# BarclayII/audiogan

Hardware: AMD Instinct MI355X
Metric: audio-samples/sec per G+D train step (8 kHz, 8192-sample clips) (higher is better)
Workload: dtype f32; 1 GPU; C2: full audiogan.py Conv1d/LSTM G + D, batch 64 per GPU, 8192-sample white-noise clips, frame_size 256 (T=32), canonical G+D step, adam, per-parameter clip d=1 g=0.1; global_batch=64, clip_len=8192, parallelism=dp1, launch=hipGraph replay (1 graph per step)

## Files before the change

### audiogan_amd/_lib.py

```python
import ctypes as C
import os

_HERE = os.path.dirname(os.path.abspath(__file__))
LIB_PATH = os.path.join(_HERE, 'libaudiogan_hip.so')

AG_OK, AG_ERR_ARG, AG_ERR_LAUNCH, AG_ERR_UNSUPPORTED = 0, -1, -2, -3
ACT_NONE, ACT_LEAKY, ACT_TANH, ACT_LEAKY_GATE = 0, 1, 2, 3
OPT_RMSPROP, OPT_ADAM = 0, 1
FLAG_NAN, FLAG_BIG = 1, 2

vp, i32, i64, f32 = C.c_void_p, C.c_int32, C.c_int64, C.c_float


class WnDesc(C.Structure):
    _fields_ = [('v', vp), ('g', vp), ('w', vp), ('wpa', vp), ('wpb', vp), ('inv_norm', vp),
                ('rows', i32), ('cols', i32), ('d1', i32), ('K', i32), ('stride', i32), ('pad_', i32)]


class WnBwdDesc(C.Structure):
    _fields_ = [('v', vp), ('g', vp), ('dw', vp), ('dv', vp), ('dg', vp), ('rows', i32), ('cols', i32),
                ('accumulate', i32), ('pad_', i32)]


class ConvArgs(C.Structure):
    _fields_ = [('x', vp), ('wp', vp), ('bias', vp), ('res', vp), ('y', vp), ('lens_i64', vp),
                ('x_bs', i64), ('x_cs', i64), ('y_bs', i64), ('y_cs', i64), ('res_bs', i64),
                ('res_cs', i64), ('B', i32), ('C', i32), ('Lin', i32), ('O', i32), ('Lout', i32),
                ('K', i32), ('stride', i32), ('pad', i32), ('mode', i32), ('act', i32),
                ('slope', f32), ('accumulate', i32), ('wp_pad', i32)]


class FrontFwdArgs(C.Structure):
    _fields_ = [('struct_bytes', i64), ('cell', i32), ('gen', i32)] + [(n, vp) for n in (
        'gates', 'gh', 'w_x', 'w_hh', 'b_hn', 'w_p', 'b_p', 'hs', 'cs', 'x', 'xt', 'w_s', 'b_s', 'u', 's', 'first', 't_run',
        'ws')] + [(n, i64) for n in ('ldx', 'lds', 'ws_bytes')] + [(n, i32) for n in ('ldwx', 'T', 'B', 'S', 'fs', 'n_cu')]


class FrontBwdArgs(C.Structure):
    _fields_ = [('struct_bytes', i64), ('cell', i32), ('pad_', i32)] + [(n, vp) for n in (
        'ga', 'state', 'gh', 'x', 'dh_ext', 'dx_ext', 'w_hh', 'w_x', 'w_p', 'dgs', 'dgh', 'dxt', 'ws')] + [
        (n, i64) for n in ('ldx', 'lddx', 'ws_bytes')] + [(n, i32) for n in ('ldwx', 'T', 'B', 'S', 'fs', 'n_cu')]


class OptDesc(C.Structure):
# ... 12 lines not shown
    'ag_abi_version': (C.c_int, []),
    'ag_bce_logits_fwd_strided': (C.c_int, [vp, i64, i64, C.c_float, vp, vp, vp, vp, C.c_float, C.c_int, C.c_int, vp]),
    'ag_bce_logits_bwd_strided': (C.c_int, [vp, i64, i64, C.c_float, vp, vp, vp, C.c_float, vp, i64, i64, C.c_int, C.c_int, vp]),
    'ag_transpose_batched': (C.c_int, [vp, C.c_int, i64, i64, vp, C.c_int, i64, i64, C.c_int, C.c_int, C.c_int, vp]),
    'ag_defer_reduces': (C.c_int, [C.c_int]),
    'ag_flush_reduces': (C.c_int, [vp]),
    'ag_arch': (C.c_char_p, []),
    'ag_last_error': (C.c_char_p, []),
    'ag_last_kernel': (C.c_char_p, []),
    'ag_weight_norm_fwd': (C.c_int, [vp, C.c_int, C.c_int, vp]),
    'ag_weight_norm_bwd': (C.c_int, [vp, C.c_int, C.c_int, vp]),
    'ag_conv1d_engine': (C.c_int, [C.POINTER(ConvArgs), vp]),
    'ag_prep_conv_weight': (C.c_int, [vp, vp, vp, C.c_int, C.c_int, C.c_int, C.c_int, C.c_int, vp]),
    'ag_wpa_numel': (i64, [C.c_int, C.c_int, C.c_int]),
    'ag_wpb_numel': (i64, [C.c_int, C.c_int, C.c_int, C.c_int]),
    'ag_conv1d_wgrad': (C.c_int, [vp, i64, i64, vp, i64, i64, vp] + [C.c_int] * 8 + [vp]),
    'ag_conv1d_o1_fwd': (C.c_int, [vp, i64, i64, vp, vp, vp, i64, C.c_int, C.c_int, C.c_int, C.c_int, C.c_int,
                                   C.c_int, f32, vp]),
    'ag_conv1d_o1_bwd_data': (C.c_int, [vp, i64, vp, vp, i64, i64, C.c_int, C.c_int, C.c_int, C.c_int, C.c_int,
                                        C.c_int, vp]),
    'ag_conv1d_o1_wgrad': (C.c_int, [vp, i64, vp, i64, i64, vp, C.c_int, C.c_int, C.c_int, C.c_int, C.c_int, vp]),
    'ag_channel_sum': (C.c_int, [vp, i64, i64, vp, C.c_int, C.c_int, C.c_int, C.c_int, vp]),
    'ag_lstm_front_bwd_step': (C.c_int, [vp, C.c_int, vp, C.c_int, vp, C.c_int, C.c_int, vp, vp, C.c_int, vp, vp, vp,
                                         vp, vp, vp, C.c_int, C.c_int, vp]),
    'ag_leaky_bwd': (C.c_int, [vp, i64, i64, vp, i64, i64, vp, i64, i64, vp, i64, i64, vp, vp, C.c_int,
                               C.c_int, C.c_int, f32, vp]),
    'ag_gemm': (C.c_int, [vp, C.c_int, C.c_int, vp, C.c_int, C.c_int, vp, C.c_int, C.c_int,
                          C.c_int, C.c_int, f32, f32, vp, vp, C.c_int, C.c_int, f32, vp]),
    'ag_col_sum': (C.c_int, [vp, C.c_int, C.c_int, vp, C.c_int, C.c_int, C.c_int, vp]),
    'ag_lstm_cell_fwd': (C.c_int, [vp, C.c_int, vp, C.c_int, vp, C.c_int, vp, C.c_int, vp, C.c_int,
# ... 100 lines not shown
```

### audiogan_amd/common.py

```python
import torch

from . import kernels as K

PARAM_EPOCH = [0]


CAPTURE_EPOCH = [0]


def new_capture():
    CAPTURE_EPOCH[0] += 1
    return CAPTURE_EPOCH[0]


def capture_tag(dev):
    if torch.device(dev).type == 'cuda' and torch.cuda.is_current_stream_capturing():
        return CAPTURE_EPOCH[0]
    return None


def param_epoch(p):
    return getattr(p, '_ag_epoch', 0)


# ... 87 lines not shown


class Prepared(object):
    __slots__ = ('w', 'wpa', 'wpb', 'pad')

    def __init__(self, w=None, wpa=None, wpb=None, pad=0):
        self.w, self.wpa, self.wpb, self.pad = w, wpa, wpb, pad


class WNGroup(object):

    def __init__(self):
        self.items = []
        self._bufs = None
        self._key = None

    def add(self, v, g, stride=1, engine=False, pad=0):
        self.items.append(dict(v=v, g=g, stride=stride, engine=engine, pad=pad))
        return len(self.items) - 1

    def params(self):
        out = []
        for it in self.items:
            out += [it['v'], it['g']]
        return out

    def _alloc(self, dev):
        bufs = []
        for it in self.items:
            v = it['v']
# ... 15 lines not shown

    def _entries(self):
        return [dict(v=it['v'].data, g=it['g'].data.view(-1), w=p.w, wpa=p.wpa, wpb=p.wpb, stride=it['stride'],
                     pad=it.get('pad', 0)) for it, p in zip(self.items, self._bufs)]

    def prepare(self):
        key = self._current_key()
        if key != self._key:
            K.weight_norm_fwd(self._entries())
            self._mark_fresh(key)
        return self._bufs

    def _mark_fresh(self, key):
        self._key = key
        self._w16 = {}

    def w16(self, i):
        d = getattr(self, '_w16', None)
        if d is None:
            d = self._w16 = {}
        img = d.get(i)
        if img is None:
            keep = getattr(self, '_w16_buf', None)
            if keep is None:
                keep = self._w16_buf = {}
            img = d[i] = K.to_bf16(self._bufs[i].w, out=keep.get(i))
            keep[i] = img
        return img

    def zero_dws(self):
# ... 79 lines not shown
```

### audiogan_amd/csrc/conv_engine.hip

```cpp
#include "conv_engine_impl.h"

int ag_conv_cfg_1214(ConvP& p, hipStream_t st);
int ag_conv_cfg_2114(ConvP& p, hipStream_t st);
int ag_conv_cfg_1122(ConvP& p, hipStream_t st);
int ag_conv_cfg_2122(ConvP& p, hipStream_t st);
int ag_conv_cfg_2222(ConvP& p, hipStream_t st);
int ag_conv_cfg_1141(ConvP& p, hipStream_t st);

extern "C" int64_t ag_wpa_numel(int d0, int d1, int K) {
  const int cp2 = ag_roundup(d1, 2), mp = ag_roundup(d0, 32);
  return ag_wq_offset(cp2, K, mp) + ag_wq_floats(cp2, K, mp);
}
extern "C" int64_t ag_wpb_numel(int d0, int d1, int K, int stride) {
  const int cp2 = ag_roundup(d0, 2), mt = ag_cdiv(K, stride), mp = ag_roundup(d1 * stride, 32);
  return ag_wq_offset(cp2, mt, mp) + ag_wq_floats(cp2, mt, mp);
}

template <typename MainFn, typename TailFn>
static int main_and_tail(hipStream_t st, MainFn mainf, TailFn tailf) {
  const int rc = mainf(st);
  if (rc != AG_OK) return rc;
  const char* main_name = ag_last_kernel();
  const int rt = tailf(st);
  ag_note_kernel(main_name);
  return rt;
}

extern "C" int ag_conv1d_engine(const ag_conv_args* args, void* stream) {
  AG_REQUIRE(args != nullptr, "ag_conv1d_engine: null args");
  ConvP p;
  p.a = *args;
  const ag_conv_args& a = p.a;
  p.aligned = 0;
  p.rb = ag_precision() == AG_PREC_BF16;
  AG_REQUIRE(a.x && a.wp && a.y, "ag_conv1d_engine: null tensor");
  AG_REQUIRE(a.B > 0 && a.C > 0 && a.O > 0 && a.Lin > 0 && a.Lout > 0, "ag_conv1d_engine: bad shape");
  AG_REQUIRE(a.K > 0 && a.stride > 0 && a.pad >= 0, "ag_conv1d_engine: bad conv params");
  AG_REQUIRE(a.B <= 65535, "ag_conv1d_engine: batch > 65535");
  AG_REQUIRE(a.mode == 0 || a.mode == 1, "ag_conv1d_engine: bad mode");
  if (a.mode == 0) {
    p.taps = a.K;
    p.sp = a.stride;
    p.Mrows = a.O;
    p.n_lo = 0;
    p.n_cnt = a.Lout;
    AG_REQUIRE((int64_t)(a.Lout - 1) * a.stride - a.pad < a.Lin, "ag_conv1d_engine: Lout too large");
  } else {
    p.taps = ag_cdiv(a.K, a.stride);
    p.sp = 1;
    p.Mrows = a.O * a.stride;
    if (a.wp_pad == a.pad && ag_scatter_aligned(a.K, a.stride, a.pad)) {
      p.aligned = 1;
      p.n_lo = ag_cdiv(a.pad, a.stride);
      p.n_cnt = ag_cdiv(a.Lout, a.stride);
    } else {
      p.n_lo = a.pad / a.stride;
      const int n_hi = (a.Lout - 1 + a.pad) / a.stride;
      p.n_cnt = n_hi - p.n_lo + 1;
    }
  }
  if (ag_conv_c1_enabled()) {
    int rc = AG_OK;
    if (ag_conv_c1_try_fwd(a, p.rb, (hipStream_t)stream, &rc)) return rc;
    if (ag_conv_c1_try_bwdx(a, p.rb, (hipStream_t)stream, &rc)) return rc;
  }
  AG_REQUIRE(p.taps <= MAX_TAPS, "ag_conv1d_engine: more than %d taps", MAX_TAPS);
  p.sp_shift = ilog2_exact(p.sp);
  p.s_shift = ilog2_exact(a.stride);
  p.efast = (int64_t)a.O * a.y_cs * 4 < ((int64_t)1 << 31) && (!a.res || (int64_t)a.O * a.res_cs * 4 < ((int64_t)1 << 31));
  p.xvec = (((uintptr_t)a.x & 15) == 0) && (a.x_bs % 4 == 0) && (a.x_cs % 4 == 0);
  p.Cpad = ag_roundup(a.C, 2);
  p.Mpad = ag_roundup(p.Mrows, 32);
  hipStream_t st = (hipStream_t)stream;
  if (p.Mrows <= 32) return ag_conv_cfg_1214(p, st);
  const int tail0 = p.n_cnt % 128;
  const int tail = (p.n_cnt - tail0) / 128 < 8 ? tail0 : 0, main_cols = p.n_cnt - tail;
  if (p.Mrows <= 64) {
    if (tail > 0 && tail <= 32 && main_cols > 0) {
      ConvP qm = p, qt = p;
      qm.n_cnt = main_cols;
      qt.n_lo += main_cols;
      qt.n_cnt = tail;
      return main_and_tail(st, [&](hipStream_t s_) { return ag_conv_cfg_2114(qm, s_); },
                           [&](hipStream_t s_) { return ag_conv_cfg_1122(qt, s_); });
// ... 51 lines not shown
}

extern "C" int ag_prep_conv_weight(const float* w, float* wpa, float* wpb, int d0, int d1, int K,
                                   int stride, int pad, void* stream) {
  AG_REQUIRE(w && (wpa || wpb), "ag_prep_conv_weight: null tensor");
  AG_REQUIRE(d0 > 0 && d1 > 0 && K > 0 && stride > 0, "ag_prep_conv_weight: bad shape");
  int64_t n = 0;
  if (wpa) n = ag_wq_offset(ag_roundup(d1, 2), K, ag_roundup(d0, 32));
  const int64_t nbw = ag_wq_offset(ag_roundup(d0, 2), ag_cdiv(K, stride), ag_roundup(d1 * stride, 32));
  if (wpb && nbw > n) n = nbw;
  hipLaunchKernelGGL(prep_conv_weight_kernel, dim3((unsigned)ag_cdiv64(n, 256)), dim3(256), 0,
                     (hipStream_t)stream, w, wpa, wpb, d0, d1, K, stride, pad);
  AG_CHECK_LAUNCH("ag_prep_conv_weight");
  return AG_OK;
}
```

### audiogan_amd/csrc/conv_engine_impl.h

```cpp
#pragma once
#include "common.h"
#include <type_traits>

#define MAX_TAPS 32

struct ConvP {
  ag_conv_args a;
  int taps;
  int sp;
  int sp_shift;
  int ncols;
  int rowlen;
  int chs;
  int CC;
  int Cpad;
  int Mrows;
  int Mpad;
  int n_lo;
  int n_cnt;
  int xvec;
  int aligned;
  int efast;
  int s_shift;
  int ncols_tile;
// ... 14 lines not shown
                                                   int b, int row0, int n0, int wrow0, int wcol0, int l31, int h) {
  const ag_conv_args& a = p.a;
  if (!p.efast) return false;
  const unsigned OOB = 0x80000000u;
  const int ycs = (int)a.y_cs, rcs = (int)a.res_cs;
  int lenb = 0x7fffffff;
  if (a.lens_i64) {
    const int64_t l = a.lens_i64[b];
    lenb = l > 0x7fffffff ? 0x7fffffff : (int)l;
  }
  __amdgpu_buffer_rsrc_t yr = __builtin_amdgcn_make_buffer_rsrc(a.y + (int64_t)b * a.y_bs, 0, (int)((int64_t)a.O * a.y_cs * 4), 0x00020000);
  __amdgpu_buffer_rsrc_t rr = __builtin_amdgcn_make_buffer_rsrc(
      const_cast<float*>(a.res ? a.res + (int64_t)b * a.res_bs : a.y), 0, a.res ? (int)((int64_t)a.O * a.res_cs * 4) : 0, 0x00020000);
  const bool has_res = a.res != nullptr;
  const bool gate = a.act == AG_ACT_LEAKY_GATE;
  if (a.mode == 0) {
#pragma unroll
    for (int i = 0; i < TILES_O; ++i) {
#pragma unroll
      for (int e = 0; e < 16; ++e) {
        const int ro = wrow0 + 32 * i + (e & 3) + 8 * (e >> 2) + 4 * h;
        const int o = row0 + ro;
        const bool valid = o < p.Mrows;
        const float bo = bias_s[ro];
        const int rowy = o * ycs, rowr = o * rcs;
#pragma unroll
        for (int j = 0; j < TILES_T; ++j) {
          const int t = n0 + wcol0 + 32 * j + l31;
          const bool ok = valid && t < a.Lout;
          const unsigned yo = ok ? (unsigned)((rowy + t) * 4) : OOB;
          float v = acc[i][j][e] + bo;
// ... 4 lines not shown
          v = ag_apply_act(v, a.act, a.slope);
          if (t >= lenb) v = 0.f;
          if (a.accumulate) v += __uint_as_float(__builtin_amdgcn_raw_buffer_load_b32(yr, yo, 0, 0));
          __builtin_amdgcn_raw_buffer_store_b32(__float_as_uint(v), yr, yo, 0, 0);
        }
      }
    }
    return true;
  }
  const int s = a.stride;
  const int rho = a.pad % s;
  const bool rot4 = p.aligned && s == 4;
  const bool al4 = p.aligned && s % 4 == 0 && rho % 4 == 0;
  const bool sw2 = p.aligned && s == 2;
  if (!sw2 && (s % 4 != 0 || (p.aligned && !rot4 && !al4))) return false;
  {
    const int nlo = n0, nhi = n0 + p.ncols_tile - 1;
    int lo, hi;
    if (sw2) { lo = 2 * nlo - a.pad - 1; hi = 2 * nhi - a.pad + 1; }
    else if (rot4) { lo = 4 * (nlo - 1) - (a.pad - rho); hi = 4 * nhi - (a.pad - rho); }
    else if (p.aligned) { lo = s * (nlo - 1) + rho - a.pad; hi = s * nhi + rho - a.pad; }
    else { lo = s * nlo - a.pad; hi = s * (nhi + 1) - a.pad; }
    if (lo < 0 || hi > a.Lout) return false;
  }
  const bool need_pre = has_res || a.accumulate;
  if (sw2) {
#pragma unroll
    for (int i = 0; i < TILES_O; ++i) {
#pragma unroll
      for (int g = 0; g < 4; ++g) {
// ... 21 lines not shown
            if (u0 >= lenb) v0 = 0.f;
            if (u0 + 1 >= lenb) v1 = 0.f;
            if (a.accumulate) {
              v0 += __uint_as_float(__builtin_amdgcn_raw_buffer_load_b32(yr, yo, 0, 0));
              v1 += __uint_as_float(__builtin_amdgcn_raw_buffer_load_b32(yr, yo + 4u, 0, 0));
            }
            __builtin_amdgcn_raw_buffer_store_b32(__float_as_uint(v0), yr, yo, 0, 0);
            __builtin_amdgcn_raw_buffer_store_b32(__float_as_uint(v1), yr, yo + 4u, 0, 0);
          }
        }
      }
    }
    return true;
  }
  const int rot = rot4 ? rho : 0;
#pragma unroll
  for (int i = 0; i < TILES_O; ++i) {
    unsigned yo[4][TILES_T];
    cu32x4 pre[4][TILES_T];
#pragma unroll
    for (int g = 0; g < 4; ++g) {
      const int rowb = row0 + wrow0 + 32 * i + 8 * g + 4 * h;
      const bool valid = rowb < p.Mrows;
      const int o = p.s_shift >= 0 ? (rowb >> p.s_shift) : rowb / s;
      const int r = rowb - o * s;
      const int rowy = o * ycs, rowr = o * rcs;
#pragma unroll
      for (int j = 0; j < TILES_T; ++j) {
        const int n = n0 + wcol0 + 32 * j + l31;
        const int u0 = rot4 ? 4 * (n - 1) - (a.pad - rho) : s * (n - ((p.aligned && r >= rho) ? 1 : 0)) + r - a.pad;
// ... 39 lines not shown
        }
        __builtin_amdgcn_raw_buffer_store_b128(out, yr, yo[g][j], 0, 0);
      }
    }
  }
  return true;
}

template <int TILES_O, int TILES_T>
__device__ __forceinline__ void conv_epilogue_any(const ConvP& p, f32x16 (&acc)[TILES_O][TILES_T], const float* bias_s,
                                                  int b, int row0, int n0, int wrow0, int wcol0, int l31, int h) {
  const ag_conv_args& a = p.a;
  const int64_t lenb = a.lens_i64 ? a.lens_i64[b] : (int64_t)1 << 60;
  float* yb = a.y + (int64_t)b * a.y_bs;
  const float* rb = a.res ? a.res + (int64_t)b * a.res_bs : nullptr;
  const int s = a.stride;
  const int rho = a.pad % s;
#pragma unroll
  for (int i = 0; i < TILES_O; ++i) {
#pragma unroll
    for (int e = 0; e < 16; ++e) {
      const int ro = wrow0 + 32 * i + (e & 3) + 8 * (e >> 2) + 4 * h;
      const int row = row0 + ro;
      if (row >= p.Mrows) continue;
      const float bo = bias_s[ro];
      const int o = a.mode == 0 ? row : row / s;
      const int r = row - o * s;
#pragma unroll
      for (int j = 0; j < TILES_T; ++j) {
        const int n = n0 + wcol0 + 32 * j + l31;
        const int u = a.mode == 0 ? n : s * (n - ((p.aligned && r >= rho) ? 1 : 0)) + r - a.pad;
        if (u < 0 || u >= a.Lout) continue;
        float v = acc[i][j][e] + bo;
        if (rb) {
          const float rv = rb[(int64_t)o * a.res_cs + u];
          v = a.act == AG_ACT_LEAKY_GATE ? (rv > 0.f ? v : v * a.slope) : v + rv;
        }
        v = ag_apply_act(v, a.act, a.slope);
        if (u >= lenb) v = 0.f;
        float* dst = yb + (int64_t)o * a.y_cs + u;
        if (a.accumulate) v += *dst;
        *dst = v;
      }
    }
  }
}

template <int TILES_O, int TILES_T>
__device__ __forceinline__ void conv_epilogue(const ConvP& p, f32x16 (&acc)[TILES_O][TILES_T], const float* bias_s,
                                              int b, int row0, int n0, int wrow0, int wcol0, int l31, int h) {
  if (!conv_epilogue_fast<TILES_O, TILES_T>(p, acc, bias_s, b, row0, n0, wrow0, wcol0, l31, h))
    conv_epilogue_any<TILES_O, TILES_T>(p, acc, bias_s, b, row0, n0, wrow0, wcol0, l31, h);
}

template <int TILES_O, int TILES_T, int WAVES_O, int WAVES_T, int TAPS, int S0>
__global__ __launch_bounds__(512) __attribute__((amdgpu_waves_per_eu(4, 4))) void conv_engine_kernel(const ConvP p) {
// ... 628 lines not shown
```

### audiogan_amd/kernels.py

```python
import ctypes as C

import torch

from . import _lib
from ._lib import lib, check, ACT_NONE, ACT_LEAKY, ACT_TANH, ACT_LEAKY_GATE, OPT_RMSPROP, OPT_ADAM

LEAKY_SLOPE = 0.01


def _stream():
    return C.c_void_p(torch.cuda.current_stream().cuda_stream)


def _p(t):
    return C.c_void_p(t.data_ptr()) if t is not None else C.c_void_p(0)


def _chk(t, name, dtype=torch.float32):
    if t is None:
        return
    if not t.is_cuda:
        raise RuntimeError('audiogan_amd: %s must be a CUDA (HIP) tensor; there is no CPU path' % name)
    if t.dtype != dtype:
        raise TypeError('audiogan_amd: %s must be %s, got %s' % (name, dtype, t.dtype))
# ... 278 lines not shown


def prep_conv_weight(w, wpa, wpb, stride, pad=0):
    _chk(w, 'w'); _chk(wpa, 'wpa'); _chk(wpb, 'wpb')
    assert w.dim() == 3 and w.is_contiguous()
    d0, d1, K = w.shape
    if wpa is not None:
        assert wpa.numel() == wpa_numel(d0, d1, K)
    if wpb is not None:
        assert wpb.numel() == wpb_numel(d0, d1, K, stride)
    check(lib.ag_prep_conv_weight(_p(w), _p(wpa), _p(wpb), d0, d1, K, stride, int(pad), _stream()),
          'ag_prep_conv_weight')


def conv_engine(x, wp, y, K, stride, pad, mode, bias=None, res=None, lens=None, act=ACT_NONE,
                slope=LEAKY_SLOPE, accumulate=False, wp_pad=0):
    assert act != ACT_LEAKY_GATE or res is not None, 'ACT_LEAKY_GATE needs the saved activation in `res`'
    x_bs, x_cs = _bcl(x, 'x')
    y_bs, y_cs = _bcl(y, 'y')
    _chk(wp, 'wp'); _chk(bias, 'bias'); _chk(lens, 'lens', torch.int64)
    B, Cc, Lin = x.shape
    B2, O, Lout = y.shape
    assert B == B2
    if mode == 0:
        assert wp.numel() == wpa_numel(O, Cc, K), 'gather weight layout does not match shapes'
    else:
        assert wp.numel() == wpb_numel(Cc, O, K, stride), 'scatter weight layout does not match'
    r_bs = r_cs = 0
    if res is not None:
        r_bs, r_cs = _bcl(res, 'res')
        assert tuple(res.shape) == tuple(y.shape)
    if bias is not None:
        assert bias.numel() == O and bias.is_contiguous()
    if lens is not None:
        assert lens.numel() == B and lens.is_contiguous()
    a = _lib.ConvArgs(x.data_ptr(), wp.data_ptr(), _p(bias).value or 0, _p(res).value or 0,
                      y.data_ptr(), _p(lens).value or 0, x_bs, x_cs, y_bs, y_cs, r_bs, r_cs,
                      B, Cc, Lin, O, Lout, K, stride, pad, mode, act, slope, 1 if accumulate else 0, int(wp_pad))
    check(lib.ag_conv1d_engine(C.byref(a), _stream()), 'ag_conv1d_engine')


def conv_wgrad(sh, lg, dw, K, stride, pad):
    sh_bs, sh_cs = _bcl(sh, 'sh')
    lg_bs, lg_cs = _bcl(lg, 'lg')
    _chk(dw, 'dw')
    B, A, Lsh = sh.shape
    B2, Cc, Llg = lg.shape
    assert B == B2 and dw.is_contiguous() and dw.numel() == A * Cc * K
    _ws = _bind_ws(lib.ag_conv1d_wgrad_ws_numel(B, A, Lsh, Cc, K), dw.device)
    check(lib.ag_conv1d_wgrad(_p(sh), sh_bs, sh_cs, _p(lg), lg_bs, lg_cs, _p(dw), B, A, Lsh, Cc, Llg,
                              K, stride, pad, _stream()), 'ag_conv1d_wgrad')


def channel_sum(dy, db, accumulate=True):
# ... 372 lines not shown
            r['bytes'] += by
        cls.records = []
        return out


def _bf16_tag():
    return '<bf16>' if lib.ag_get_precision() == 1 else ''


def _work_gemm(A, B, Cm, ta=False, tb=False, *a_, **kw):
    M, N = Cm.shape
    Kd = A.size(0) if ta else A.size(1)
    return None, 2.0 * M * N * Kd, 4.0 * (M * Kd + N * Kd + M * N)


def _work_conv(x, wp, y, K_, stride, pad, mode, *a_, **kw):
    B, Cc, Lin = x.shape
    _, O, Lout = y.shape
    macs = B * O * Lout * Cc * K_ if mode == 0 else B * Cc * Lin * O * K_
    return None, 2.0 * macs, 4.0 * (x.numel() + y.numel() + O * Cc * K_)


def _work_wgrad(sh, lg, dw, K_, stride, pad):
    B, A, Lsh = sh.shape
    Cc = lg.size(1)
    return None, 2.0 * B * A * Lsh * Cc * K_, 4.0 * (sh.numel() + lg.numel() + dw.numel())


def _call_sig(a, k):
    def one(v):
        if isinstance(v, torch.Tensor):
            return tuple(v.shape), v.stride(), v.dtype, v.data_ptr() % 16
        if isinstance(v, (list, tuple)):
            return tuple(one(e) for e in v)
        return v
# ... 20 lines not shown
        e0, e1 = torch.cuda.Event(enable_timing=True), torch.cuda.Event(enable_timing=True)
        e0.record()
        r = fn(*a, **k)
        e1.record()
        if key is None:
            key = seen[sig] = lib.ag_last_kernel().decode()
        Profiler.records.append((key, fl, by, e0, e1, nl))
        return r
    wrapped.__name__ = name
    wrapped.__doc__ = fn.__doc__
    wrapped.__module__ = __name__
    globals()[name] = wrapped


for _n, _w in (('gemm', _work_gemm), ('conv_engine', _work_conv), ('conv_wgrad', _work_wgrad),
               ('channel_sum', None), ('leaky_bwd', None), ('col_sum', None), ('lstm_cell_fwd', None),
               ('lstm_cell_bwd', None), ('weight_norm_fwd', None), ('weight_norm_bwd', None),
               ('bce_logits_fwd', None), ('bce_logits_bwd', None), ('act_fwd', None), ('act_bwd', None),
               ('axpby', None), ('grad_norms', None), ('opt_step', None)):
    _instrument(_n, _w)


def _al16(t):
    return t.data_ptr() % 16 == 0


def skinny_ok(A, B, tb):
    M, Kd = A.shape
    ok = M <= 256 and Kd % 8 == 0 and A.stride(1) == 1 and A.stride(0) % 4 == 0 and _al16(A)
    if tb:
        ok = ok and B.stride(1) == 1 and B.stride(0) % 4 == 0 and _al16(B)
# ... 753 lines not shown
```

### audiogan_amd/ops.py

```python
import torch

from . import kernels as K
from .kernels import ACT_NONE, ACT_LEAKY, ACT_TANH, ACT_LEAKY_GATE

from .common import PARAM_EPOCH, Prepared, WNGroup, _zeros_like_list


class ConvSpec(object):
    __slots__ = ('kind', 'cin', 'cout', 'K', 'stride', 'pad', 'out_pad')

    def __init__(self, kind, cin, cout, K_, stride, pad, out_pad=0):
        self.kind, self.cin, self.cout, self.K, self.stride, self.pad = kind, cin, cout, K_, stride, pad
        self.out_pad = out_pad

    def out_len(self, lin):
        if self.kind == 'conv':
            return (lin + 2 * self.pad - self.K) // self.stride + 1
        return (lin - 1) * self.stride - 2 * self.pad + self.K + self.out_pad


def _o1(spec):
    return K.conv_o1_ok(spec.kind, spec.cout, spec.K, spec.stride, spec.pad)


# ... 17 lines not shown
    else:
        K.conv_engine(dy, prep.wpa, dx, spec.K, spec.stride, spec.pad, 0, res=gate, lens=lens, act=act, accumulate=accumulate)


def conv_wgrad(spec, x, dy, dw, db):
    if _o1(spec):
        K.conv_o1_wgrad(dy, x, dw, spec.K, spec.pad)
    elif spec.kind == 'conv':
        K.conv_wgrad(dy, x, dw, spec.K, spec.stride, spec.pad)
    else:
        K.conv_wgrad(x, dy, dw, spec.K, spec.stride, spec.pad)
    if db is not None:
        K.channel_sum(dy, db)


class GTrunk(object):

    def __init__(self, bottlenecks, final):
        self.bottlenecks = bottlenecks
        self.final = final
        self.group = WNGroup()
        self.ctot = 1 + sum(d.cout for _, d in bottlenecks)


class GTrunkFn(torch.autograd.Function):
    @staticmethod
    def forward(ctx, x0, trunk, *params):
        B, L = x0.shape
        prep = trunk.group.prepare()
        ctot = trunk.ctot
        if (x0.stride() == (ctot * L, 1) and x0.storage_offset() == 0 and x0.dtype == torch.float32
                and x0.untyped_storage().nbytes() == 4 * B * ctot * L):
            slab = x0.as_strided((B, ctot, L), (ctot * L, L, 1), 0)
        else:
            slab = torch.empty(B, ctot, L, device=x0.device)
            slab[:, 0, :].copy_(x0)
        hids = []
# ... 26 lines not shown
        dy = dy.contiguous().view(B, 1, L)
        wg = any(ctx.needs_input_grad[2:])
        dws = trunk.group.zero_dws() if wg else None
        dslab = torch.empty_like(slab)
        with K.deferred_reduces():
            GTrunkFn._backward_layers(trunk, prep, slab, hids, dy, dslab, dws, wg, ctot)
        grads = trunk.group.backward(dws) if wg else [None] * (2 * len(trunk.group.items))
        dx0 = dslab[:, 0, :] if ctx.needs_input_grad[0] else None
        return (dx0, None) + tuple(grads)

    @staticmethod
    def _backward_layers(trunk, prep, slab, hids, dy, dslab, dws, wg, ctot):
        if wg:
            conv_wgrad(trunk.final, slab, dy, dws[-2], dws[-1])
        conv_bwd_data(trunk.final, prep[-2], dy, dslab, accumulate=False)
        cin = ctot
        for i in reversed(range(len(trunk.bottlenecks))):
            cs, ds = trunk.bottlenecks[i]
            pw, qw = prep[4 * i], prep[4 * i + 2]
            cin -= ds.cout
            out_v = slab[:, cin:cin + ds.cout]
            dout = dslab[:, cin:cin + ds.cout]
            add = dslab[:, cin - ds.cout:cin] if cin >= ds.cout else None
            K.leaky_bwd(dout, out_v, dout, add_into=add, bias_grad=dws[4 * i + 3] if wg else None)
            hid = hids[i]
            if wg:
                conv_wgrad(ds, hid, dout, dws[4 * i + 2], None)
            dhid = torch.empty_like(hid)
            conv_bwd_data(ds, qw, dout, dhid, gate=hid)
            if wg:
                K.channel_sum(dhid, dws[4 * i + 1])
            if wg:
                conv_wgrad(cs, slab[:, :cin], dhid, dws[4 * i], None)
            conv_bwd_data(cs, pw, dhid, dslab[:, :cin], accumulate=True)


class DConvStack(object):
    def __init__(self, specs):
        self.specs = specs
        self.group = WNGroup()


class DConvStackFn(torch.autograd.Function):

    @staticmethod
    def forward(ctx, x, stack, lens_list, *params):
        B, L = x.shape
        ctx.set_materialize_grads(False)
        prep = stack.group.prepare()
# ... 307 lines not shown
```

### include/audiogan_hip.h

```cpp
#ifndef AUDIOGAN_HIP_H
#define AUDIOGAN_HIP_H

#include <stdint.h>

#ifdef __cplusplus
extern "C" {
#endif

#define AG_OK 0
#define AG_ERR_ARG (-1)
#define AG_ERR_LAUNCH (-2)
#define AG_ERR_UNSUPPORTED (-3)

#define AG_ACT_NONE 0
#define AG_ACT_LEAKY 1
#define AG_ACT_TANH 2
#define AG_ACT_LEAKY_GATE 3

int ag_abi_version(void);
const char* ag_arch(void);
const char* ag_last_error(void);
const char* ag_last_kernel(void);

typedef struct ag_wn_desc {
// ... 15 lines not shown

typedef struct ag_wn_bwd_desc {
  const float* v;
  const float* g;
  const float* dw;
  float* dv;
  float* dg;
  int32_t rows;
  int32_t cols;
  int32_t accumulate;
  int32_t pad_;
} ag_wn_bwd_desc;

int ag_weight_norm_bwd(const ag_wn_bwd_desc* descs_dev, int n, int max_rows, void* stream);

typedef struct ag_conv_args {
  const float* x;
  const float* wp;
  const float* bias;
  const float* res;
  float* y;
  const int64_t* lens_i64;
  int64_t x_bs, x_cs;
  int64_t y_bs, y_cs;
  int64_t res_bs, res_cs;
  int32_t B, C, Lin, O, Lout;
  int32_t K, stride, pad;
  int32_t mode;
  int32_t act;
  float slope;
  int32_t accumulate;
  int32_t wp_pad;
} ag_conv_args;

int ag_conv1d_engine(const ag_conv_args* args, void* stream);

int ag_prep_conv_weight(const float* w, float* wpa, float* wpb, int d0, int d1, int K, int stride, int pad,
                        void* stream);
int64_t ag_wpa_numel(int d0, int d1, int K);
int64_t ag_wpb_numel(int d0, int d1, int K, int stride);

int ag_conv1d_wgrad(const float* sh, int64_t sh_bs, int64_t sh_cs, const float* lg, int64_t lg_bs,
                    int64_t lg_cs, float* dw, int B, int A, int Lsh, int C, int Llg, int K,
                    int stride, int pad, void* stream);

int ag_conv1d_o1_fwd(const float* x, int64_t x_bs, int64_t x_cs, const float* w, const float* bias, float* y,
                     int64_t y_bs, int B, int C, int L, int K, int pad, int act, float slope, void* stream);
int ag_conv1d_o1_bwd_data(const float* dy, int64_t dy_bs, const float* w, float* dx, int64_t dx_bs,
                          int64_t dx_cs, int B, int C, int L, int K, int pad, int accumulate, void* stream);
int ag_conv1d_o1_wgrad(const float* dy, int64_t dy_bs, const float* x, int64_t x_bs, int64_t x_cs, float* dw,
                       int B, int C, int L, int K, int pad, void* stream);

int ag_channel_sum(const float* dy, int64_t bs, int64_t cs, float* db, int B, int C, int L, int accumulate,
                   void* stream);

// ... 237 lines not shown
```

Measured before the change: 31.03 million audio-samples/sec.

## Pull dense-trunk input gradients via concatenated weight panels in generator backward

Restructures the generator dense-trunk backward. Each bottleneck used to scatter its input-gradient conv into the growing slab, followed by a separate leaky backward. Now per-slice weight panels are built from all later bottlenecks (rebuilt when weights change), and one conv per output slice pulls the hidden gradients of every later layer. The leaky gate, residual add and pre-accumulate are fused into that conv's epilogue. This cuts repeated read-modify-write passes over the gradient slab and launches, at the cost of extra panel memory, a pull kernel per weight refresh and a new epilogue path that bypasses the c1 fast path.

```diff
diff --git a/audiogan_amd/_lib.py b/audiogan_amd/_lib.py
--- a/audiogan_amd/_lib.py
+++ b/audiogan_amd/_lib.py
@@ -6,6 +6,7 @@
 
 AG_OK, AG_ERR_ARG, AG_ERR_LAUNCH, AG_ERR_UNSUPPORTED = 0, -1, -2, -3
 ACT_NONE, ACT_LEAKY, ACT_TANH, ACT_LEAKY_GATE = 0, 1, 2, 3
+CONV_ACC_POST, CONV_ACC_PRE = 1, 2
 OPT_RMSPROP, OPT_ADAM = 0, 1
 FLAG_NAN, FLAG_BIG = 1, 2
 
@@ -27,7 +28,13 @@
                 ('x_bs', i64), ('x_cs', i64), ('y_bs', i64), ('y_cs', i64), ('res_bs', i64),
                 ('res_cs', i64), ('B', i32), ('C', i32), ('Lin', i32), ('O', i32), ('Lout', i32),
                 ('K', i32), ('stride', i32), ('pad', i32), ('mode', i32), ('act', i32),
-                ('slope', f32), ('accumulate', i32), ('wp_pad', i32)]
+                ('slope', f32), ('accumulate', i32), ('wp_pad', i32), ('gate_from', i32), ('add', vp),
+                ('add_bs', i64), ('add_cs', i64)]
+
+
+class PullDesc(C.Structure):
+    _fields_ = [('src', vp), ('dst', vp), ('C', i32), ('taps', i32), ('src_mp', i32), ('row0', i32), ('rows', i32),
+                ('dst_mp', i32), ('c0', i32), ('ctot', i32)]
 
 
 class FrontFwdArgs(C.Structure):
@@ -70,6 +77,7 @@
     'ag_prep_conv_weight': (C.c_int, [vp, vp, vp, C.c_int, C.c_int, C.c_int, C.c_int, C.c_int, vp]),
     'ag_wpa_numel': (i64, [C.c_int, C.c_int, C.c_int]),
     'ag_wpb_numel': (i64, [C.c_int, C.c_int, C.c_int, C.c_int]),
+    'ag_pull_panels': (C.c_int, [vp, C.c_int, i64, vp]),
     'ag_conv1d_wgrad': (C.c_int, [vp, i64, i64, vp, i64, i64, vp] + [C.c_int] * 8 + [vp]),
     'ag_conv1d_o1_fwd': (C.c_int, [vp, i64, i64, vp, vp, vp, i64, C.c_int, C.c_int, C.c_int, C.c_int, C.c_int,
                                    C.c_int, f32, vp]),
diff --git a/audiogan_amd/common.py b/audiogan_amd/common.py
--- a/audiogan_amd/common.py
+++ b/audiogan_amd/common.py
@@ -125,6 +125,7 @@
         self.items = []
         self._bufs = None
         self._key = None
+        self.derived = None
 
     def add(self, v, g, stride=1, engine=False, pad=0):
         self.items.append(dict(v=v, g=g, stride=stride, engine=engine, pad=pad))
@@ -170,6 +171,9 @@
     def _mark_fresh(self, key):
         self._key = key
         self._w16 = {}
+        derived = getattr(self, 'derived', None)
+        if derived is not None:
+            derived(self._bufs)
 
     def w16(self, i):
         d = getattr(self, '_w16', None)
diff --git a/audiogan_amd/csrc/conv_engine.hip b/audiogan_amd/csrc/conv_engine.hip
--- a/audiogan_amd/csrc/conv_engine.hip
+++ b/audiogan_amd/csrc/conv_engine.hip
@@ -38,6 +38,10 @@
   AG_REQUIRE(a.K > 0 && a.stride > 0 && a.pad >= 0, "ag_conv1d_engine: bad conv params");
   AG_REQUIRE(a.B <= 65535, "ag_conv1d_engine: batch > 65535");
   AG_REQUIRE(a.mode == 0 || a.mode == 1, "ag_conv1d_engine: bad mode");
+  AG_REQUIRE(a.accumulate >= 0 && a.accumulate <= AG_CONV_ACC_PRE, "ag_conv1d_engine: bad accumulate");
+  AG_REQUIRE(a.gate_from >= 0 && a.gate_from <= a.O, "ag_conv1d_engine: gate_from outside the output channels");
+  AG_REQUIRE(a.gate_from == 0 || a.act == AG_ACT_NONE || a.act == AG_ACT_LEAKY_GATE,
+             "ag_conv1d_engine: gate_from needs AG_ACT_LEAKY_GATE or AG_ACT_NONE");
   if (a.mode == 0) {
     p.taps = a.K;
     p.sp = a.stride;
@@ -59,7 +63,7 @@
       p.n_cnt = n_hi - p.n_lo + 1;
     }
   }
-  if (ag_conv_c1_enabled()) {
+  if (ag_conv_c1_enabled() && !a.add) {
     int rc = AG_OK;
     if (ag_conv_c1_try_fwd(a, p.rb, (hipStream_t)stream, &rc)) return rc;
     if (ag_conv_c1_try_bwdx(a, p.rb, (hipStream_t)stream, &rc)) return rc;
@@ -67,7 +71,8 @@
   AG_REQUIRE(p.taps <= MAX_TAPS, "ag_conv1d_engine: more than %d taps", MAX_TAPS);
   p.sp_shift = ilog2_exact(p.sp);
   p.s_shift = ilog2_exact(a.stride);
-  p.efast = (int64_t)a.O * a.y_cs * 4 < ((int64_t)1 << 31) && (!a.res || (int64_t)a.O * a.res_cs * 4 < ((int64_t)1 << 31));
+  p.efast = (int64_t)a.O * a.y_cs * 4 < ((int64_t)1 << 31) && (!a.res || (int64_t)a.O * a.res_cs * 4 < ((int64_t)1 << 31)) &&
+            (!a.add || (int64_t)a.O * a.add_cs * 4 < ((int64_t)1 << 31));
   p.xvec = (((uintptr_t)a.x & 15) == 0) && (a.x_bs % 4 == 0) && (a.x_cs % 4 == 0);
   p.Cpad = ag_roundup(a.C, 2);
   p.Mpad = ag_roundup(p.Mrows, 32);
@@ -149,3 +154,25 @@
   AG_CHECK_LAUNCH("ag_prep_conv_weight");
   return AG_OK;
 }
+
+__global__ __launch_bounds__(256) void pull_panels_kernel(const ag_pull_desc* __restrict__ descs) {
+  const ag_pull_desc d = descs[blockIdx.y];
+  const int64_t i = (int64_t)blockIdx.x * 256 + threadIdx.x;
+  if (i >= (int64_t)d.C * d.taps * d.dst_mp) return;
+  const int row = (int)(i % d.dst_mp);
+  const int cm = (int)(i / d.dst_mp);
+  const int m = cm % d.taps, c = cm / d.taps;
+  const float val = row < d.rows ? d.src[(int64_t)cm * d.src_mp + d.row0 + row] : 0.f;
+  d.dst[((int64_t)(d.c0 + c) * d.taps + m) * d.dst_mp + row] = val;
+  unsigned short* q = reinterpret_cast<unsigned short*>(d.dst + ag_wq_offset((d.ctot + 1) & ~1, d.taps, d.dst_mp));
+  q[ag_wq_index(d.c0 + c, m, row, d.taps, d.dst_mp)] = (unsigned short)ag_pack_bf16(val, val);
+}
+
+extern "C" int ag_pull_panels(const ag_pull_desc* descs_dev, int n, int64_t max_elems, void* stream) {
+  AG_REQUIRE(descs_dev && n > 0 && max_elems > 0, "ag_pull_panels: bad args");
+  AG_REQUIRE(n <= 65535, "ag_pull_panels: too many descriptors");
+  hipLaunchKernelGGL(pull_panels_kernel, dim3((unsigned)ag_cdiv64(max_elems, 256), n), dim3(256), 0,
+                     (hipStream_t)stream, descs_dev);
+  AG_CHECK_LAUNCH("ag_pull_panels");
+  return AG_OK;
+}
diff --git a/audiogan_amd/csrc/conv_engine_impl.h b/audiogan_amd/csrc/conv_engine_impl.h
--- a/audiogan_amd/csrc/conv_engine_impl.h
+++ b/audiogan_amd/csrc/conv_engine_impl.h
@@ -52,7 +52,9 @@
       const_cast<float*>(a.res ? a.res + (int64_t)b * a.res_bs : a.y), 0, a.res ? (int)((int64_t)a.O * a.res_cs * 4) : 0, 0x00020000);
   const bool has_res = a.res != nullptr;
   const bool gate = a.act == AG_ACT_LEAKY_GATE;
+  const bool pull = a.accumulate == AG_CONV_ACC_PRE || a.add != nullptr || a.gate_from > 0;
   if (a.mode == 0) {
+    if (pull) return false;
 #pragma unroll
     for (int i = 0; i < TILES_O; ++i) {
 #pragma unroll
@@ -87,6 +89,7 @@
   const bool al4 = p.aligned && s % 4 == 0 && rho % 4 == 0;
   const bool sw2 = p.aligned && s == 2;
   if (!sw2 && (s % 4 != 0 || (p.aligned && !rot4 && !al4))) return false;
+  if (sw2 && pull) return false;
   {
     const int nlo = n0, nhi = n0 + p.ncols_tile - 1;
     int lo, hi;
@@ -138,6 +141,76 @@
     return true;
   }
   const int rot = rot4 ? rho : 0;
+  if (pull) {
+    __amdgpu_buffer_rsrc_t ar = __builtin_amdgcn_make_buffer_rsrc(
+        const_cast<float*>(a.add ? a.add + (int64_t)b * a.add_bs : a.y), 0, a.add ? (int)((int64_t)a.O * a.add_cs * 4) : 0, 0x00020000);
+    const int acs = (int)a.add_cs;
+    const bool has_add = a.add != nullptr;
+    const bool acc_pre = a.accumulate == AG_CONV_ACC_PRE, acc_post = a.accumulate == AG_CONV_ACC_POST;
+    const cu32x4 zero4 = {0u, 0u, 0u, 0u};
+#pragma unroll
+    for (int i = 0; i < TILES_O; ++i) {
+#pragma unroll
+      for (int gh = 0; gh < 2; ++gh) {
+        unsigned yo[2][TILES_T];
+        cu32x4 pr[2][TILES_T], py[2][TILES_T], pa[2][TILES_T];
+#pragma unroll
+        for (int g2 = 0; g2 < 2; ++g2) {
+          const int rowb = row0 + wrow0 + 32 * i + 8 * (2 * gh + g2) + 4 * h;
+          const bool valid = rowb < p.Mrows;
+          const int o = p.s_shift >= 0 ? (rowb >> p.s_shift) : rowb / s;
+          const int r = rowb - o * s;
+#pragma unroll
+          for (int j = 0; j < TILES_T; ++j) {
+            const int n = n0 + wcol0 + 32 * j + l31;
+            const int u0 = rot4 ? 4 * (n - 1) - (a.pad - rho) : s * (n - ((p.aligned && r >= rho) ? 1 : 0)) + r - a.pad;
+            yo[g2][j] = valid ? (unsigned)((o * ycs + u0) * 4) : OOB;
+            pr[g2][j] = has_res ? __builtin_amdgcn_raw_buffer_load_b128(rr, valid ? (unsigned)((o * rcs + u0) * 4) : OOB, 0, 0) : zero4;
+            py[g2][j] = a.accumulate ? __builtin_amdgcn_raw_buffer_load_b128(yr, yo[g2][j], 0, 0) : zero4;
+            pa[g2][j] = has_add ? __builtin_amdgcn_raw_buffer_load_b128(ar, valid ? (unsigned)((o * acs + u0) * 4) : OOB, 0, 0) : zero4;
+          }
+        }
+#pragma unroll
+        for (int g2 = 0; g2 < 2; ++g2) {
+          const int g = 2 * gh + g2;
+          const int ro = wrow0 + 32 * i + 8 * g + 4 * h;
+          const int rowb = row0 + ro;
+          const int o = p.s_shift >= 0 ? (rowb >> p.s_shift) : rowb / s;
+          const int r = rowb - o * s;
+          const float bo = bias_s[ro];
+          const bool gated = o >= a.gate_from;
+#pragma unroll
+          for (int j = 0; j < TILES_T; ++j) {
+            const int n = n0 + wcol0 + 32 * j + l31;
+            const int u0 = rot4 ? 4 * (n - 1) - (a.pad - rho) : s * (n - ((p.aligned && r >= rho) ? 1 : 0)) + r - a.pad;
+            const float v4[4] = {acc[i][j][4 * g], acc[i][j][4 * g + 1], acc[i][j][4 * g + 2], acc[i][j][4 * g + 3]};
+            float v[4];
+            if (rot == 0) { v[0] = v4[0]; v[1] = v4[1]; v[2] = v4[2]; v[3] = v4[3]; }
+            else if (rot == 1) { v[0] = v4[1]; v[1] = v4[2]; v[2] = v4[3]; v[3] = v4[0]; }
+            else if (rot == 2) { v[0] = v4[2]; v[1] = v4[3]; v[2] = v4[0]; v[3] = v4[1]; }
+            else { v[0] = v4[3]; v[1] = v4[0]; v[2] = v4[1]; v[3] = v4[2]; }
+            cu32x4 out;
+#pragma unroll
+            for (int q = 0; q < 4; ++q) {
+              const float rv = __uint_as_float(pr[g2][j][q]), ov = __uint_as_float(py[g2][j][q]);
+              float w = v[q] + bo;
+              if (has_res && !gate) w += rv;
+              if (acc_pre) w += ov;
+              if (has_add) w += __uint_as_float(pa[g2][j][q]);
+              if (gated) {
+                w = gate ? (rv > 0.f ? w : w * a.slope) : ag_apply_act(w, a.act, a.slope);
+                if (u0 + q >= lenb) w = 0.f;
+              }
+              if (acc_post) w += ov;
+              out[q] = __float_as_uint(w);
+            }
+            __builtin_amdgcn_raw_buffer_store_b128(out, yr, yo[g2][j], 0, 0);
+          }
+        }
+      }
+    }
+    return true;
+  }
 #pragma unroll
   for (int i = 0; i < TILES_O; ++i) {
     unsigned yo[4][TILES_T];
@@ -207,6 +280,8 @@
   const int64_t lenb = a.lens_i64 ? a.lens_i64[b] : (int64_t)1 << 60;
   float* yb = a.y + (int64_t)b * a.y_bs;
   const float* rb = a.res ? a.res + (int64_t)b * a.res_bs : nullptr;
+  const float* ab = a.add ? a.add + (int64_t)b * a.add_bs : nullptr;
+  const bool gate = a.act == AG_ACT_LEAKY_GATE;
   const int s = a.stride;
   const int rho = a.pad % s;
 #pragma unroll
@@ -225,14 +300,16 @@
         const int u = a.mode == 0 ? n : s * (n - ((p.aligned && r >= rho) ? 1 : 0)) + r - a.pad;
         if (u < 0 || u >= a.Lout) continue;
         float v = acc[i][j][e] + bo;
-        if (rb) {
-          const float rv = rb[(int64_t)o * a.res_cs + u];
-          v = a.act == AG_ACT_LEAKY_GATE ? (rv > 0.f ? v : v * a.slope) : v + rv;
-        }
-        v = ag_apply_act(v, a.act, a.slope);
-        if (u >= lenb) v = 0.f;
         float* dst = yb + (int64_t)o * a.y_cs + u;
-        if (a.accumulate) v += *dst;
+        const float rv = rb ? rb[(int64_t)o * a.res_cs + u] : 0.f;
+        if (rb && !gate) v += rv;
+        if (a.accumulate == AG_CONV_ACC_PRE) v += *dst;
+        if (ab) v += ab[(int64_t)o * a.add_cs + u];
+        if (o >= a.gate_from) {
+          v = gate ? (rv > 0.f ? v : v * a.slope) : ag_apply_act(v, a.act, a.slope);
+          if (u >= lenb) v = 0.f;
+        }
+        if (a.accumulate == AG_CONV_ACC_POST) v += *dst;
         *dst = v;
       }
     }
diff --git a/audiogan_amd/kernels.py b/audiogan_amd/kernels.py
--- a/audiogan_amd/kernels.py
+++ b/audiogan_amd/kernels.py
@@ -4,6 +4,7 @@
 
 from . import _lib
 from ._lib import lib, check, ACT_NONE, ACT_LEAKY, ACT_TANH, ACT_LEAKY_GATE, OPT_RMSPROP, OPT_ADAM
+from ._lib import CONV_ACC_POST, CONV_ACC_PRE
 
 LEAKY_SLOPE = 0.01
 
@@ -316,7 +317,7 @@
 
 
 def conv_engine(x, wp, y, K, stride, pad, mode, bias=None, res=None, lens=None, act=ACT_NONE,
-                slope=LEAKY_SLOPE, accumulate=False, wp_pad=0):
+                slope=LEAKY_SLOPE, accumulate=False, wp_pad=0, add=None, gate_from=0):
     assert act != ACT_LEAKY_GATE or res is not None, 'ACT_LEAKY_GATE needs the saved activation in `res`'
     x_bs, x_cs = _bcl(x, 'x')
     y_bs, y_cs = _bcl(y, 'y')
@@ -336,10 +337,32 @@
         assert bias.numel() == O and bias.is_contiguous()
     if lens is not None:
         assert lens.numel() == B and lens.is_contiguous()
+    a_bs = a_cs = 0
+    if add is not None:
+        a_bs, a_cs = _bcl(add, 'add')
+        assert tuple(add.shape) == tuple(y.shape)
+    assert 0 <= gate_from <= O and (gate_from == 0 or act in (ACT_NONE, ACT_LEAKY_GATE))
     a = _lib.ConvArgs(x.data_ptr(), wp.data_ptr(), _p(bias).value or 0, _p(res).value or 0,
                       y.data_ptr(), _p(lens).value or 0, x_bs, x_cs, y_bs, y_cs, r_bs, r_cs,
-                      B, Cc, Lin, O, Lout, K, stride, pad, mode, act, slope, 1 if accumulate else 0, int(wp_pad))
+                      B, Cc, Lin, O, Lout, K, stride, pad, mode, act, slope, int(accumulate), int(wp_pad),
+                      int(gate_from), _p(add).value or 0, a_bs, a_cs)
     check(lib.ag_conv1d_engine(C.byref(a), _stream()), 'ag_conv1d_engine')
+
+
+def pull_panels(entries):
+    descs, nmax = [], 1
+    for e in entries:
+        _chk(e['src'], 'src'); _chk(e['dst'], 'dst')
+        Cc, taps, smp, dmp, ctot = e['C'], e['taps'], e['src_mp'], e['dst_mp'], e['ctot']
+        cp2 = (ctot + 1) // 2 * 2
+        assert 0 <= e['row0'] and e['row0'] + e['rows'] <= smp and e['rows'] <= dmp and e['c0'] + Cc <= ctot
+        assert e['src'].numel() >= Cc * taps * smp, 'source layout smaller than its descriptor'
+        assert e['dst'].numel() == cp2 * taps * dmp + (cp2 + 15) // 16 * 16 * taps * dmp // 2, 'panel size'
+        descs.append(_lib.PullDesc(e['src'].data_ptr(), e['dst'].data_ptr(), Cc, taps, smp, e['row0'], e['rows'], dmp,
+                                   e['c0'], ctot))
+        nmax = max(nmax, Cc * taps * dmp)
+    tab = _table('pull', descs, entries[0]['src'].device)
+    check(lib.ag_pull_panels(_p(tab), len(descs), nmax, _stream()), 'ag_pull_panels')
 
 
 def conv_wgrad(sh, lg, dw, K, stride, pad):
@@ -742,11 +765,13 @@
     return None, 2.0 * M * N * Kd, 4.0 * (M * Kd + N * Kd + M * N)
 
 
-def _work_conv(x, wp, y, K_, stride, pad, mode, *a_, **kw):
+def _work_conv(x, wp, y, K_, stride, pad, mode, bias=None, res=None, lens=None, act=ACT_NONE, slope=LEAKY_SLOPE,
+               accumulate=False, wp_pad=0, add=None, gate_from=0):
     B, Cc, Lin = x.shape
     _, O, Lout = y.shape
     macs = B * O * Lout * Cc * K_ if mode == 0 else B * Cc * Lin * O * K_
-    return None, 2.0 * macs, 4.0 * (x.numel() + y.numel() + O * Cc * K_)
+    ny = y.numel() * (1 + (1 if accumulate else 0) + (1 if add is not None else 0))
+    return None, 2.0 * macs, 4.0 * (x.numel() + ny + O * Cc * K_)
 
 
 def _work_wgrad(sh, lg, dw, K_, stride, pad):
@@ -797,7 +822,7 @@
 
 
 for _n, _w in (('gemm', _work_gemm), ('conv_engine', _work_conv), ('conv_wgrad', _work_wgrad),
-               ('channel_sum', None), ('leaky_bwd', None), ('col_sum', None), ('lstm_cell_fwd', None),
+               ('channel_sum', None), ('leaky_bwd', None), ('pull_panels', None), ('col_sum', None), ('lstm_cell_fwd', None),
                ('lstm_cell_bwd', None), ('weight_norm_fwd', None), ('weight_norm_bwd', None),
                ('bce_logits_fwd', None), ('bce_logits_bwd', None), ('act_fwd', None), ('act_bwd', None),
                ('axpby', None), ('grad_norms', None), ('opt_step', None)):
diff --git a/audiogan_amd/ops.py b/audiogan_amd/ops.py
--- a/audiogan_amd/ops.py
+++ b/audiogan_amd/ops.py
@@ -55,6 +55,54 @@
         K.channel_sum(dy, db)
 
 
+class PullStep(object):
+    __slots__ = ('o0', 'o1', 'src', 'gate_from', 'add')
+
+    def __init__(self, o0, o1, src, gate_from, add):
+        self.o0, self.o1, self.src = o0, o1, src
+        self.gate_from = gate_from
+        self.add = add
+
+
+def pull_plan(bottlenecks):
+    n = len(bottlenecks)
+    if n < 2:
+        return None
+    cins = [1]
+    for _, d in bottlenecks:
+        cins.append(cins[-1] + d.cout)
+
+    def key(i):
+        c = bottlenecks[i][0]
+        return (c.kind, c.K, c.stride, c.pad)
+
+    def skip(i):
+        return cins[i] >= bottlenecks[i][1].cout
+
+    def exact(i):
+        return i >= 1 and bottlenecks[i][1].cout == bottlenecks[i - 1][1].cout
+
+    if key(n - 1)[0] != 'conv':
+        return None
+    lo = n - 1
+    while lo >= 1 and key(lo - 1) == key(n - 1) and (not skip(lo - 1) or exact(lo - 1)):
+        lo -= 1
+    if n - lo < 2:
+        return None
+    steps = {}
+    for i in range(n - 1, lo, -1):
+        add = skip(i) and exact(i)
+        steps[i] = [PullStep(cins[i - 1], cins[i], i, 0, add)]
+    pre = lo >= 1 and not skip(lo - 1)
+    if lo >= 1 and skip(lo):
+        w = cins[lo] - cins[lo - 1]
+        steps[lo] = [PullStep(cins[lo - 1], cins[lo], lo, 0 if pre else w, True),
+                     PullStep(0, cins[lo - 1], lo, cins[lo - 1], False)]
+    else:
+        steps[lo] = [PullStep(0, cins[lo], lo, cins[lo - 1] if pre else cins[lo], False)]
+    return lo, steps, (lo - 1 if pre else lo)
+
+
 class GTrunk(object):
 
     def __init__(self, bottlenecks, final):
@@ -62,6 +110,47 @@
         self.final = final
         self.group = WNGroup()
         self.ctot = 1 + sum(d.cout for _, d in bottlenecks)
+        self.pull = pull_plan(bottlenecks)
+        self.panels = {}
+        if self.pull is not None:
+            self.group.derived = self._build_panels
+
+    def hid_offsets(self):
+        lo, offs, o = self.pull[0], {}, 0
+        for i in range(lo, len(self.bottlenecks)):
+            offs[i] = o
+            o += self.bottlenecks[i][0].cout
+        return offs, o
+
+    def pull_on(self, t):
+        plan = getattr(self, 'pull', None)
+        return plan if t.is_cuda else None
+
+    def _build_panels(self, bufs):
+        lo, steps = self.pull[:2]
+        if self.pull_on(bufs[4 * lo].wpb) is None:
+            return
+        n = len(self.bottlenecks)
+        offs, htot = self.hid_offsets()
+        cs0 = self.bottlenecks[lo][0]
+        s, taps = cs0.stride, (cs0.K + cs0.stride - 1) // cs0.stride
+        ents = []
+        for i in steps:
+            for st in steps[i]:
+                ctot = htot - offs[st.src]
+                pkey = (st.o0, st.o1, st.src)
+                dev = bufs[4 * lo].wpb.device
+                pan = self.panels.get(pkey)
+                if pan is None or pan.device != dev:
+                    pan = self.panels[pkey] = torch.zeros(K.wpb_numel(ctot, st.o1 - st.o0, cs0.K, s), device=dev)
+                dst_mp = ((st.o1 - st.o0) * s + 31) // 32 * 32
+                for j in range(st.src, n):
+                    cj = self.bottlenecks[j][0]
+                    assert bufs[4 * j].pad == bufs[4 * lo].pad
+                    ents.append(dict(src=bufs[4 * j].wpb, dst=pan, C=cj.cout, taps=taps, src_mp=(cj.cin * s + 31) // 32 * 32,
+                                     row0=st.o0 * s, rows=(st.o1 - st.o0) * s, dst_mp=dst_mp, c0=offs[j] - offs[st.src],
+                                     ctot=ctot))
+        K.pull_panels(ents)
 
 
 class GTrunkFn(torch.autograd.Function):
@@ -118,25 +207,46 @@
         if wg:
             conv_wgrad(trunk.final, slab, dy, dws[-2], dws[-1])
         conv_bwd_data(trunk.final, prep[-2], dy, dslab, accumulate=False)
+        n = len(trunk.bottlenecks)
+        plan = trunk.pull_on(slab)
+        lo, steps, first = plan if plan is not None else (n, {}, n)
+        if plan is not None:
+            offs, htot = trunk.hid_offsets()
+            dhid_all = torch.empty(slab.size(0), htot, hids[lo].size(2), device=slab.device)
         cin = ctot
-        for i in reversed(range(len(trunk.bottlenecks))):
+        for i in reversed(range(n)):
             cs, ds = trunk.bottlenecks[i]
             pw, qw = prep[4 * i], prep[4 * i + 2]
             cin -= ds.cout
             out_v = slab[:, cin:cin + ds.cout]
             dout = dslab[:, cin:cin + ds.cout]
-            add = dslab[:, cin - ds.cout:cin] if cin >= ds.cout else None
-            K.leaky_bwd(dout, out_v, dout, add_into=add, bias_grad=dws[4 * i + 3] if wg else None)
+            if first <= i < n - 1:
+                if wg:
+                    K.channel_sum(dout, dws[4 * i + 3])
+            else:
+                add = dslab[:, cin - ds.cout:cin] if cin >= ds.cout else None
+                if i >= lo and steps[i][0].add:
+                    add = None
+                K.leaky_bwd(dout, out_v, dout, add_into=add, bias_grad=dws[4 * i + 3] if wg else None)
             hid = hids[i]
             if wg:
                 conv_wgrad(ds, hid, dout, dws[4 * i + 2], None)
-            dhid = torch.empty_like(hid)
+            dhid = dhid_all[:, offs[i]:offs[i] + cs.cout] if i >= lo else torch.empty_like(hid)
             conv_bwd_data(ds, qw, dout, dhid, gate=hid)
             if wg:
                 K.channel_sum(dhid, dws[4 * i + 1])
             if wg:
                 conv_wgrad(cs, slab[:, :cin], dhid, dws[4 * i], None)
-            conv_bwd_data(cs, pw, dhid, dslab[:, :cin], accumulate=True)
+            if i < lo:
+                conv_bwd_data(cs, pw, dhid, dslab[:, :cin], accumulate=True)
+                continue
+            for st in steps[i]:
+                width = st.o1 - st.o0
+                gated = st.gate_from < width
+                K.conv_engine(dhid_all[:, offs[st.src]:], trunk.panels[(st.o0, st.o1, st.src)], dslab[:, st.o0:st.o1],
+                              cs.K, cs.stride, cs.pad, 1, res=slab[:, st.o0:st.o1] if gated else None,
+                              act=ACT_LEAKY_GATE if gated else ACT_NONE, accumulate=K.CONV_ACC_PRE, wp_pad=pw.pad,
+                              add=dout if st.add else None, gate_from=st.gate_from if gated else 0)
 
 
 class DConvStack(object):
diff --git a/include/audiogan_hip.h b/include/audiogan_hip.h
--- a/include/audiogan_hip.h
+++ b/include/audiogan_hip.h
@@ -53,6 +53,8 @@
 
 int ag_weight_norm_bwd(const ag_wn_bwd_desc* descs_dev, int n, int max_rows, void* stream);
 
+#define AG_CONV_ACC_POST 1
+#define AG_CONV_ACC_PRE 2
 typedef struct ag_conv_args {
   const float* x;
   const float* wp;
@@ -70,6 +72,9 @@
   float slope;
   int32_t accumulate;
   int32_t wp_pad;
+  int32_t gate_from;
+  const float* add;
+  int64_t add_bs, add_cs;
 } ag_conv_args;
 
 int ag_conv1d_engine(const ag_conv_args* args, void* stream);
@@ -78,6 +83,14 @@
                         void* stream);
 int64_t ag_wpa_numel(int d0, int d1, int K);
 int64_t ag_wpb_numel(int d0, int d1, int K, int stride);
+
+typedef struct ag_pull_desc {
+  const float* src;
+  float* dst;
+  int32_t C, taps, src_mp, row0, rows, dst_mp, c0, ctot;
+} ag_pull_desc;
+
+int ag_pull_panels(const ag_pull_desc* descs_dev, int n, int64_t max_elems, void* stream);
 
 int ag_conv1d_wgrad(const float* sh, int64_t sh_bs, int64_t sh_cs, const float* lg, int64_t lg_bs,
                     int64_t lg_cs, float* dw, int B, int A, int Lsh, int C, int Llg, int K,
```

New measurement: 31.06 million audio-samples/sec, median of 5. Within noise of the previous version (+0.1%).
